# DreamScene-Project/DreamScene

Measured on AMD Instinct MI355X. Metric: fwd+bwd views/s @1024x1024, 500000 Gaussians, higher is better.
Workload: dtype f32

## Files before the change

dreamscene_amd/csrc/render.hip:

```cpp
#include "gsr_common.h"
#include <cstdlib>

namespace {

constexpr int kBatch = 256;

__device__ __forceinline__ float gsr_mul(float a, float b) {
#pragma clang fp contract(off)
  return a * b;
}
__device__ __forceinline__ float gsr_sub(float a, float b) {
#pragma clang fp contract(off)
  return a - b;
}
__device__ __forceinline__ float gsr_exp(float x) {
  const float t = gsr_mul(x, 1.44269502162933349609375f);
  const float n = __builtin_rintf(t);
  const float f = gsr_sub(t, n);
  float p = 0.001326472731307149f;
  p = __fmaf_rn(p, f, 0.009671512991189957f);
  p = __fmaf_rn(p, f, 0.05550733581185341f);
  p = __fmaf_rn(p, f, 0.24022242426872253f);
  p = __fmaf_rn(p, f, 0.6931470036506653f);
  p = __fmaf_rn(p, f, 1.0f);
  return __builtin_amdgcn_ldexpf(p, gsr_f2i_sat_fast(n));
}
__device__ __forceinline__ float gsr_power(float hA, float nB, float hC, float dx, float dy) {
  return __fmaf_rn(dx, __fmaf_rn(hA, dx, gsr_mul(nB, dy)), gsr_mul(gsr_mul(hC, dy), dy));
}

struct TilePix {
  int px, py, bx, by;
  bool inside;
};

__device__ __forceinline__ TilePix tile_pixel(int tile, int gx, int W, int H) {
  const int tid = threadIdx.x, wave = tid >> 6, lane = tid & 63;
  const int ty = tile / gx, tx = tile - ty * gx;
  TilePix p;
  p.bx = tx * GSR_TILE + (wave & 1) * 8;
  p.by = ty * GSR_TILE + (wave >> 1) * 8;
  p.px = p.bx + (lane & 7);
  p.py = p.by + (lane >> 3);
  p.inside = (p.px < W) && (p.py < H);
  return p;
}

template <int W1>
__device__ __forceinline__ bool block_reach(float A, float C, float B2, float nBiA, float nBiC, float tau, float cx,
                                            float cy, float bx, float by) {
  const float dx1 = cx - bx, dx0 = dx1 - (float)(W1 - 1), dy1 = cy - by, dy0 = dy1 - (float)(W1 - 1);
  const float ex = __builtin_amdgcn_fmed3f(dx0, 0.f, dx1), ey = __builtin_amdgcn_fmed3f(dy0, 0.f, dy1);
  const float y = __builtin_amdgcn_fmed3f(dy0, nBiC * ex, dy1);
  const float q1 = A * ex * ex + (B2 * ex + C * y) * y;
  const float x = __builtin_amdgcn_fmed3f(dx0, nBiA * ey, dx1);
  const float q2 = C * ey * ey + (B2 * ey + A * x) * x;
  return fminf(q1, q2) <= tau;
}

template <int W1>
__device__ __forceinline__ uint32_t block_mask_t(const float4 q0, const float4 q1, const float4 q2, int x0i, int y0i) {
  const float tau = q2.z;
  if (!(tau >= 0.f)) return 0u;
  const float A = q0.z, B = q0.w, C = q1.x;
  const float nBiA = -B * __builtin_amdgcn_rcpf(A), nBiC = -B * __builtin_amdgcn_rcpf(C), B2 = 2.f * B;
  const float x0 = (float)x0i, y0 = (float)y0i;
  uint32_t m = 0;
  m |= (uint32_t)block_reach<W1>(A, C, B2, nBiA, nBiC, tau, q0.x, q0.y, x0, y0);
  m |= (uint32_t)block_reach<W1>(A, C, B2, nBiA, nBiC, tau, q0.x, q0.y, x0 + (float)W1, y0) << 1;
  m |= (uint32_t)block_reach<W1>(A, C, B2, nBiA, nBiC, tau, q0.x, q0.y, x0, y0 + (float)W1) << 2;
  m |= (uint32_t)block_reach<W1>(A, C, B2, nBiA, nBiC, tau, q0.x, q0.y, x0 + (float)W1, y0 + (float)W1) << 3;
  return m;
}

template <int CTRL>
__device__ __forceinline__ int gsr_dpp_i(int v) {
  return __builtin_amdgcn_update_dpp(0, v, CTRL, 0xF, 0xF, true);
}

__device__ __forceinline__ uint32_t block_excl_scan_1024(uint32_t x, uint32_t* wave_tot, uint32_t* carry_s, bool update) {
  const int tid = threadIdx.x, lane = tid & 63, wave = tid >> 6;
  uint32_t inc = x;
#pragma unroll
  for (int o = 1; o < 64; o <<= 1) {
    const uint32_t t = (uint32_t)__shfl_up((int)inc, o, 64);
    if (lane >= o) inc += t;
  }
  if (lane == 63) wave_tot[wave] = inc;
  __syncthreads();
  uint32_t woff = 0;
  for (int w = 0; w < wave; ++w) woff += wave_tot[w];
  const uint32_t carry = *carry_s;
  const uint32_t excl = carry + woff + inc - x;
  __syncthreads();
  if (update && tid == 1023) *carry_s = carry + woff + inc;
  __syncthreads();
  return excl;
}

struct WorkFwdViews {
  const uint32_t* ranges[GSR_MAX_BATCH_VIEWS];
  uint32_t* tile_depth[GSR_MAX_BATCH_VIEWS];
  uint32_t* work[GSR_MAX_BATCH_VIEWS];
  uint32_t* stats_host[GSR_MAX_BATCH_VIEWS];
};
struct WorkBwdViews {
  const uint32_t* tile_depth[GSR_MAX_BATCH_VIEWS];
  uint32_t* items[GSR_MAX_BATCH_VIEWS];
  uint32_t items_cap[GSR_MAX_BATCH_VIEWS];
  uint32_t seg_len[GSR_MAX_BATCH_VIEWS];
};

#ifndef GSR_ORDER_FRAC_BITS
#define GSR_ORDER_FRAC_BITS 2
#endif
constexpr int kOrderFrac = GSR_ORDER_FRAC_BITS;
constexpr int kOrderClasses = 2 + (32 << kOrderFrac);
__device__ __forceinline__ uint32_t order_class(uint32_t len) {
  if (len == 0u) return 0u;
  const int msb = 31 - __clz(len);
  if constexpr (kOrderFrac == 0) return (uint32_t)msb + 1u;
  const uint32_t frac = (msb >= kOrderFrac ? (len >> (msb - kOrderFrac)) : (len << (kOrderFrac - msb))) & ((1u << kOrderFrac) - 1u);
  return 1u + ((uint32_t)msb << kOrderFrac) + frac;
}
__global__ void __launch_bounds__(1024)
k_work_order_fwd(const uint32_t n_tiles, const WorkFwdViews wv) {
  const uint32_t* __restrict__ ranges = wv.ranges[blockIdx.x];
  uint32_t* __restrict__ tile_depth = wv.tile_depth[blockIdx.x];
  uint32_t* __restrict__ work = wv.work[blockIdx.x];
  uint32_t* __restrict__ stats_host = wv.stats_host[blockIdx.x];
  __shared__ uint32_t cnt[kOrderClasses], cur[kOrderClasses];
  const int tid = threadIdx.x;
  if (tid < kOrderClasses) cnt[tid] = 0;
  __syncthreads();
  for (uint32_t t = tid; t < n_tiles; t += 1024) {
    const uint32_t len = ranges[2 * t + 1] - ranges[2 * t];
    atomicAdd(&cnt[order_class(len)], 1u);
    tile_depth[t] = 0;
  }
  __syncthreads();
  if (tid == 0) {
    uint32_t run = 0;
    for (int b = kOrderClasses - 1; b >= 0; --b) { cur[b] = run; run += cnt[b]; }
    work[n_tiles] = n_tiles - cnt[0];
    if (stats_host) *stats_host = n_tiles - cnt[0];
  }
  __syncthreads();
  for (uint32_t t = tid; t < n_tiles; t += 1024) {
    const uint32_t len = ranges[2 * t + 1] - ranges[2 * t];
    work[atomicAdd(&cur[order_class(len)], 1u)] = t;
  }
}

__global__ void __launch_bounds__(1024)
k_work_order_bwd(const uint32_t n_tiles, const WorkBwdViews wv) {
  const uint32_t* __restrict__ tile_depth = wv.tile_depth[blockIdx.x];
  uint32_t* __restrict__ items = wv.items[blockIdx.x];
  const uint32_t items_cap = wv.items_cap[blockIdx.x];
  const uint32_t kb = wv.seg_len[blockIdx.x];
  __shared__ uint32_t cnt[32], cur[32];
  const int tid = threadIdx.x;
  if (tid < 32) cnt[tid] = 0;
  __syncthreads();
  for (uint32_t t = tid; t < n_tiles; t += 1024) {
    const uint32_t d = tile_depth[t];
    if (d == 0) continue;
    const uint32_t full = d / kb, tail = d % kb;
    for (uint32_t sgi = 0; sgi < full; ++sgi) atomicAdd(&cnt[15u - min(15u, (d - kb * sgi - 1u) >> 8)], 1u);
    if (tail) atomicAdd(&cnt[16u + 15u - ((tail - 1u) * 16u) / kb], 1u);
  }
  __syncthreads();
  if (tid == 0) {
    uint32_t run = 0;
    for (int b = 0; b < 32; ++b) { cur[b] = run; run += cnt[b]; }
    items[0] = min(run, items_cap);
  }
  __syncthreads();
  for (uint32_t t = tid; t < n_tiles; t += 1024) {
    const uint32_t d = tile_depth[t];
    if (d == 0) continue;
    const uint32_t full = d / kb, tail = d % kb;
    for (uint32_t sgi = 0; sgi < full; ++sgi) {
      const uint32_t i = atomicAdd(&cur[15u - min(15u, (d - kb * sgi - 1u) >> 8)], 1u);
      if (i < items_cap) { items[2 + 2 * i] = t; items[3 + 2 * i] = sgi; }
    }
    if (tail) {
      const uint32_t i = atomicAdd(&cur[16u + 15u - ((tail - 1u) * 16u) / kb], 1u);
      if (i < items_cap) { items[2 + 2 * i] = t; items[3 + 2 * i] = full; }
    }
  }
}

template <bool SCORE, int PAD = 0>
struct Stage {
  float4 s0[2][kBatch + PAD], s1[2][kBatch + PAD], s2[2][kBatch + PAD];
  uint32_t sid[SCORE ? 2 : 1][SCORE ? kBatch : 1];
  uint32_t cnt[SCORE ? 2 : 1][SCORE ? kBatch : 1];
};
__device__ __forceinline__ uint32_t stage_mask(const float4& s2row) { return __float_as_uint(s2row.w); }

template <bool SCORE, int KB>
__device__ __forceinline__ void
render_fwd_body(const uint32_t item, const int W, const int H, const uint32_t* __restrict__ work, float* __restrict__ ckpt,
             const uint32_t* __restrict__ ranges,
             const uint32_t* __restrict__ point_list, const float4* __restrict__ splat, const float* __restrict__ bg,
             float* __restrict__ out_color, float* __restrict__ out_da, float* __restrict__ final_T,
             uint32_t* __restrict__ n_contrib, uint32_t* __restrict__ tile_depth, float* __restrict__ score,
             const int score_mode) {
  __shared__ Stage<SCORE, 1> st;
  __shared__ uint16_t cand[4][kBatch + 16];
  if (threadIdx.x < 2) {
    st.s0[threadIdx.x][kBatch] = make_float4(0.f, 0.f, 0.f, 0.f);
    st.s1[threadIdx.x][kBatch] = make_float4(0.f, 0.f, 0.f, 0.f);
    st.s2[threadIdx.x][kBatch] = make_float4(0.f, 0.f, 0.f, 0.f);
  }
  if constexpr (SCORE) { st.cnt[0][threadIdx.x] = 0u; st.cnt[1][threadIdx.x] = 0u; }
  auto flush_counts = [&](const int b) {
    if constexpr (SCORE) {
      const uint32_t c = st.cnt[b][threadIdx.x];
      if (c) {
        atomicAdd(reinterpret_cast<uint32_t*>(score) + st.sid[b][threadIdx.x], c);
        st.cnt[b][threadIdx.x] = 0u;
      }
    }
  };
  const int gx = (W + GSR_TILE - 1) / GSR_TILE;
  const int tid = threadIdx.x, wave = tid >> 6, lane = tid & 63;
  const int slot = (lane >> 2) & 3, pcol = lane & 3, prow = lane >> 4;
  const float bg0 = bg[0], bg1 = bg[1], bg2 = bg[2];
  {
    const uint32_t tile = work[item >> 2];
    const int quarter = (int)(item & 3u);
    const int ty = (int)tile / gx, tx = (int)tile - ty * gx;
    const int q_x0 = tx * GSR_TILE + (quarter & 1) * 8, q_y0 = ty * GSR_TILE + (quarter >> 1) * 8;
    const int px = q_x0 + (wave & 1) * 4 + pcol, py = q_y0 + (wave >> 1) * 4 + prow;
    const bool inside = (px < W) && (py < H);
    const float pxf = (float)px, pyf = (float)py;
    const uint32_t r0 = ranges[2 * tile], r1 = ranges[2 * tile + 1];
    if (r0 == r1) {
      if (quarter == 0) {
        const int ex = tx * GSR_TILE + (tid & 15), ey = ty * GSR_TILE + (tid >> 4);
        if (ex < W && ey < H) {
          const size_t pix = (size_t)ey * W + ex, HW = (size_t)H * W;
          final_T[pix] = 1.0f;
          n_contrib[pix] = 0u;
          out_color[pix] = bg0; out_color[HW + pix] = bg1; out_color[2 * HW + pix] = bg2;
          out_da[pix] = 0.f; out_da[HW + pix] = 0.f;
        }
      }
      return;
    }

    unsigned long long donem = __builtin_amdgcn_ballot_w64(!inside);
    float T = 1.0f, C0 = 0.f, C1 = 0.f, C2 = 0.f, Dp = 0.f, Wt = 0.f;
    uint32_t last = 0;

    uint32_t nid = 0;
    float4 n0 = make_float4(0, 0, 0, 0), n1 = n0, n2 = n0;
    if (r0 + tid < r1) {
      nid = point_list[r0 + tid];
      const float4* r = splat + 3 * (size_t)nid;
      n0 = r[0]; n1 = r[1]; n2 = r[2];
    }
    int buf = 0;
    for (uint32_t base = r0; base < r1; base += kBatch, buf ^= 1) {
      const int n = (int)min((uint32_t)kBatch, r1 - base);
      st.s0[buf][tid] = make_float4(n0.x, n0.y, -0.5f * n0.z, -n0.w);
      st.s1[buf][tid] = make_float4(-0.5f * n1.x, n1.y, n1.z, n1.w);
      st.s2[buf][tid] = make_float4(n2.x, n2.y, n2.z,
                                    __uint_as_float((tid < n) ? block_mask_t<4>(n0, n1, n2, q_x0, q_y0) : 0u));
      if constexpr (SCORE) st.sid[buf][tid] = nid;
      const int n_done = __syncthreads_count(__builtin_amdgcn_inverse_ballot_w64(donem));
      if (score_mode != 1 && base != r0) flush_counts(buf ^ 1);
      if (n_done == 256) break;
      auto checkpoint = [&](const uint32_t pos) {
        if (ckpt == nullptr) return;
        float f0 = C0, f1 = C1, f2 = C2, f3 = Dp, f4 = Wt;
        f0 += gsr_dpp<0x124>(f0); f0 += gsr_dpp<0x128>(f0);
        f1 += gsr_dpp<0x124>(f1); f1 += gsr_dpp<0x128>(f1);
        f2 += gsr_dpp<0x124>(f2); f2 += gsr_dpp<0x128>(f2);
        f3 += gsr_dpp<0x124>(f3); f3 += gsr_dpp<0x128>(f3);
        f4 += gsr_dpp<0x124>(f4); f4 += gsr_dpp<0x128>(f4);
        if (slot == 0 && inside) {
          float* ck = ckpt + (size_t)(pos / KB) * (6 * 256) + ((py - ty * GSR_TILE) * GSR_TILE + (px - tx * GSR_TILE));
          ck[0] = T; ck[256] = f0; ck[512] = f1; ck[768] = f2; ck[1024] = f3; ck[1280] = f4;
        }
      };
      if (base != r0) checkpoint(base);
      {
        const uint32_t idx = base + kBatch + tid;
        if (idx < r1) {
          nid = point_list[idx];
          const float4* r = splat + 3 * (size_t)nid;
          n0 = r[0]; n1 = r[1]; n2 = r[2];
        }
      }
      int cnt = 0;
      int cut_at[3] = {-1, -1, -1};
#pragma unroll
      for (int k = 0; k < kBatch / 64; ++k) {
        if (k * 64 >= n) break;
        const bool m = (stage_mask(st.s2[buf][k * 64 + lane]) >> wave) & 1u;
        const unsigned long long bal = __builtin_amdgcn_ballot_w64(m);
        if (m) cand[wave][cnt + (int)__builtin_amdgcn_mbcnt_hi((uint32_t)(bal >> 32), __builtin_amdgcn_mbcnt_lo((uint32_t)bal, 0u))] = (uint8_t)(k * 64 + lane);
        cnt += (int)__popcll(bal);
        if constexpr (KB < kBatch) {
          if (((k + 1) * 64) % KB == 0 && k + 1 < kBatch / 64 && (k + 1) * 64 < n) {
            const int pad = (-cnt) & 3;
            if (lane < pad) cand[wave][cnt + lane] = (uint16_t)kBatch;
            cnt += pad;
            cut_at[(k + 1) * 64 / KB - 1] = cnt;
          }
        }
      }
      if (lane < 3) cand[wave][cnt + lane] = (uint16_t)kBatch;
      __builtin_amdgcn_fence(__ATOMIC_ACQ_REL, "wavefront");
      __builtin_amdgcn_wave_barrier();
      {
        for (int i = 0;; i += 4) {
          if (donem == ~0ull) break;
          if constexpr (KB < kBatch) {
#pragma unroll
            for (int c = 0; c < kBatch / KB - 1; ++c)
              if (i == cut_at[c]) checkpoint(base + (uint32_t)((c + 1) * KB));
          }
          if (i >= cnt) break;
          const int j = (int)cand[wave][i + slot];
          const float4 a = st.s0[buf][j];
          const float4 b = st.s1[buf][j];
          const float2 c = *reinterpret_cast<const float2*>(&st.s2[buf][j]);
          const float dx = a.x - pxf, dy = a.y - pyf;
          const float power = gsr_power(a.z, a.w, b.x, dx, dy);
          const float alpha = fminf(GSR_ALPHA_MAX, gsr_mul(b.y, gsr_exp(power)));
          const unsigned long long gm = ~donem & __builtin_amdgcn_ballot_w64(power <= 0.0f) &
                                        __builtin_amdgcn_ballot_w64(alpha >= GSR_ALPHA_MIN);
          const bool g = __builtin_amdgcn_inverse_ballot_w64(gm);
          const float fgate = g ? gsr_sub(1.0f, alpha) : 1.0f;
          float test_T = gsr_mul(T, fgate);
          asm("s_nop 1\n\t"
              "v_mul_f32_dpp %0, %0, %1 row_shr:4 row_mask:0xf bank_mask:0xe\n\t"
              "s_nop 1\n\t"
              "v_mul_f32_dpp %0, %0, %1 row_shr:4 row_mask:0xf bank_mask:0xc\n\t"
              "s_nop 1\n\t"
              "v_mul_f32_dpp %0, %0, %1 row_shr:4 row_mask:0xf bank_mask:0x8"
              : "+v"(test_T) : "v"(fgate));
          float w_all = alpha * T;
          asm("s_nop 1\n\t"
              "v_mul_f32_dpp %0, %1, %2 row_shr:4 row_mask:0xf bank_mask:0xe"
              : "+v"(w_all) : "v"(test_T), "v"(alpha));
          const unsigned long long stopm = __builtin_amdgcn_ballot_w64(test_T < GSR_T_MIN);
          const bool hit = __builtin_amdgcn_inverse_ballot_w64(gm & ~stopm);
          const float w = hit ? w_all : 0.0f;
          C0 = fmaf(b.w, w, C0); C1 = fmaf(c.x, w, C1); C2 = fmaf(c.y, w, C2);
          Dp = fmaf(b.z, w, Dp);
          Wt += w;
          last = hit ? ((base - r0) + (uint32_t)j + 1u) : last;
          if constexpr (SCORE) {
            const unsigned long long hm = __ballot(hit) & (0x000F000F000F000Full << (4 * slot));
            if (score_mode != 1) {
              if (hm != 0ull && lane == 4 * slot) atomicAdd(&st.cnt[buf][j & (kBatch - 1)], (uint32_t)__popcll(hm));
            } else {
              float ws = w;
              ws += gsr_dpp<0xB1>(ws);
              ws += gsr_dpp<0x4E>(ws);
              ws += __shfl_xor(ws, 16, 64);
              ws += __shfl_xor(ws, 32, 64);
              if (hm != 0ull && lane == 4 * slot) unsafeAtomicAdd(score + st.sid[buf][j & (kBatch - 1)], ws);
            }
          }
          uint32_t tn = __float_as_uint(hit ? test_T : T);
          tn = min(tn, (uint32_t)gsr_dpp_i<0x124>((int)tn));
          tn = min(tn, (uint32_t)gsr_dpp_i<0x128>((int)tn));
          T = __uint_as_float(tn);
          unsigned long long quad_stop = (stopm >> 12) & 0x000F000F000F000Full;
          quad_stop |= quad_stop << 4;
          quad_stop |= quad_stop << 8;
          donem |= quad_stop;
        }
      }
    }
    if constexpr (SCORE) {
      __syncthreads();
      if (score_mode != 1) flush_counts(buf ^ 1);
    }
    C0 += gsr_dpp<0x124>(C0); C0 += gsr_dpp<0x128>(C0);
    C1 += gsr_dpp<0x124>(C1); C1 += gsr_dpp<0x128>(C1);
    C2 += gsr_dpp<0x124>(C2); C2 += gsr_dpp<0x128>(C2);
    Dp += gsr_dpp<0x124>(Dp); Dp += gsr_dpp<0x128>(Dp);
    Wt += gsr_dpp<0x124>(Wt); Wt += gsr_dpp<0x128>(Wt);
    {
      int l = (int)last;
      l = max(l, gsr_dpp_i<0x124>(l));
      l = max(l, gsr_dpp_i<0x128>(l));
      last = (uint32_t)l;
    }
    if (inside && slot == 0) {
      const size_t pix = (size_t)py * W + px, HW = (size_t)H * W;
      final_T[pix] = T;
      n_contrib[pix] = last;
      out_color[pix] = C0 + T * bg0;
      out_color[HW + pix] = C1 + T * bg1;
      out_color[2 * HW + pix] = C2 + T * bg2;
      out_da[pix] = Dp;
      out_da[HW + pix] = Wt;
    }
    const uint32_t wm = gsr_wave_max_u32(last);
    if (lane == 0 && wm) atomicMax(tile_depth + tile, wm);
  }
}

template <bool SCORE>
__device__ __forceinline__ void
render_fwd_tile_body(const uint32_t item, const int W, const int H, const uint32_t* __restrict__ work, float* __restrict__ ckpt,
                  const uint32_t* __restrict__ ranges, const uint32_t* __restrict__ point_list,
                  const float4* __restrict__ splat, const float* __restrict__ bg, float* __restrict__ out_color,
                  float* __restrict__ out_da, float* __restrict__ final_T, uint32_t* __restrict__ n_contrib,
                  uint32_t* __restrict__ tile_depth, float* __restrict__ score, const int score_mode) {
  __shared__ Stage<SCORE> st;
  const int gx = (W + GSR_TILE - 1) / GSR_TILE;
  const int tile = (int)work[item];
  const int tid = threadIdx.x, wave = tid >> 6, lane = tid & 63;
  const TilePix p = tile_pixel(tile, gx, W, H);
  const int tile_x0 = p.bx - (wave & 1) * 8, tile_y0 = p.by - (wave >> 1) * 8;
  const float pxf = (float)p.px, pyf = (float)p.py;
  const uint32_t r0 = ranges[2 * tile], r1 = ranges[2 * tile + 1];
  unsigned long long donem = __builtin_amdgcn_ballot_w64(!p.inside);
  float T = 1.0f, C0 = 0.f, C1 = 0.f, C2 = 0.f, Dp = 0.f, Wt = 0.f;
  uint32_t last = 0;
  uint32_t nid = 0;
  float4 n0 = make_float4(0, 0, 0, 0), n1 = n0, n2 = n0;
  if (r0 + tid < r1) {
    nid = point_list[r0 + tid];
    const float4* r = splat + 3 * (size_t)nid;
    n0 = r[0]; n1 = r[1]; n2 = r[2];
  }
  int buf = 0;
  for (uint32_t base = r0; base < r1; base += kBatch, buf ^= 1) {
    const int n = (int)min((uint32_t)kBatch, r1 - base);
    st.s0[buf][tid] = make_float4(n0.x, n0.y, -0.5f * n0.z, -n0.w);
    st.s1[buf][tid] = make_float4(-0.5f * n1.x, n1.y, n1.z, n1.w);
    st.s2[buf][tid] = make_float4(n2.x, n2.y, n2.z,
                                  __uint_as_float((tid < n) ? block_mask_t<8>(n0, n1, n2, tile_x0, tile_y0) : 0u));
    if constexpr (SCORE) st.sid[buf][tid] = nid;
    if (__syncthreads_count(__builtin_amdgcn_inverse_ballot_w64(donem)) == 256) break;
    if (base != r0 && p.inside && ckpt != nullptr) {
      float* ck = ckpt + (size_t)(base / kBatch) * (6 * 256) + ((p.py - tile_y0) * GSR_TILE + (p.px - tile_x0));
      ck[0] = T; ck[256] = C0; ck[512] = C1; ck[768] = C2; ck[1024] = Dp; ck[1280] = Wt;
    }
    {
      const uint32_t idx = base + kBatch + tid;
      if (idx < r1) {
        nid = point_list[idx];
        const float4* r = splat + 3 * (size_t)nid;
        n0 = r[0]; n1 = r[1]; n2 = r[2];
      }
    }
    for (int k = 0; k < kBatch / 64; ++k) {
      if (k * 64 >= n) break;
      unsigned long long bits = __ballot((stage_mask(st.s2[buf][k * 64 + lane]) >> wave) & 1u);
      while (bits) {
        if (donem == ~0ull) break;
        const int j = k * 64 + __builtin_ctzll(bits);
        bits &= bits - 1ull;
        const float4 a = st.s0[buf][j];
        const float4 b = st.s1[buf][j];
        const float4 c = st.s2[buf][j];
        const float dx = a.x - pxf, dy = a.y - pyf;
        const float power = gsr_power(a.z, a.w, b.x, dx, dy);
        const float alpha = fminf(GSR_ALPHA_MAX, gsr_mul(b.y, gsr_exp(power)));
        const float test_T = gsr_mul(T, gsr_sub(1.0f, alpha));
        const unsigned long long gm = ~donem & __builtin_amdgcn_ballot_w64(power <= 0.0f) &
                                      __builtin_amdgcn_ballot_w64(alpha >= GSR_ALPHA_MIN);
        const unsigned long long stopm = gm & __builtin_amdgcn_ballot_w64(test_T < GSR_T_MIN);
        donem |= stopm;
        const bool hit = __builtin_amdgcn_inverse_ballot_w64(gm & ~stopm);
        const float w = hit ? alpha * T : 0.0f;
        if constexpr (SCORE) {
          const unsigned long long hm = __ballot(hit);
          if (hm) {
            if (score_mode != 1) {
              if (lane == 0) atomicAdd(reinterpret_cast<uint32_t*>(score) + st.sid[buf][j], (uint32_t)__popcll(hm));
            } else {
              float sc = gsr_wave_sum_to_lane63(w);
              sc = __shfl(sc, 63, 64);
              if (lane == 0) unsafeAtomicAdd(score + st.sid[buf][j], sc);
            }
          }
        }
        C0 = fmaf(b.w, w, C0); C1 = fmaf(c.x, w, C1); C2 = fmaf(c.y, w, C2);
        Dp = fmaf(b.z, w, Dp);
        Wt += w;
        T = hit ? test_T : T;
        last = hit ? ((base - r0) + (uint32_t)j + 1u) : last;
      }
    }
  }
  if (p.inside) {
    const size_t pix = (size_t)p.py * W + p.px, HW = (size_t)H * W;
    final_T[pix] = T;
    n_contrib[pix] = last;
    out_color[pix] = C0 + T * bg[0];
    out_color[HW + pix] = C1 + T * bg[1];
    out_color[2 * HW + pix] = C2 + T * bg[2];
    out_da[pix] = Dp;
    out_da[HW + pix] = Wt;
  }
  const uint32_t wm = gsr_wave_max_u32(last);
  if (lane == 0 && wm) atomicMax(tile_depth + tile, wm);
}

__device__ __forceinline__ float add_swap32(float a, float b) {
  const auto r = __builtin_amdgcn_permlane32_swap(__float_as_uint(a), __float_as_uint(b), false, false);
  return __uint_as_float(r[0]) + __uint_as_float(r[1]);
}
__device__ __forceinline__ float add_swap16(float a, float b) {
  const auto r = __builtin_amdgcn_permlane16_swap(__float_as_uint(a), __float_as_uint(b), false, false);
  return __uint_as_float(r[0]) + __uint_as_float(r[1]);
}
__device__ __forceinline__ float reduce10(const float v[10], int lane) {
  float p0, p1, p2, p3, p4, q0, q1, q2;
  asm("s_nop 1\n\t"
      "v_add_f32_dpp %0, %8, %8 row_ror:8 row_mask:0xf bank_mask:0x3\n\t"
      "v_add_f32_dpp %0, %9, %9 row_ror:8 row_mask:0xf bank_mask:0xc\n\t"
      "v_add_f32_dpp %1, %10, %10 row_ror:8 row_mask:0xf bank_mask:0x3\n\t"
      "v_add_f32_dpp %1, %11, %11 row_ror:8 row_mask:0xf bank_mask:0xc\n\t"
      "v_add_f32_dpp %2, %12, %12 row_ror:8 row_mask:0xf bank_mask:0x3\n\t"
      "v_add_f32_dpp %2, %13, %13 row_ror:8 row_mask:0xf bank_mask:0xc\n\t"
      "v_add_f32_dpp %3, %14, %14 row_ror:8 row_mask:0xf bank_mask:0x3\n\t"
      "v_add_f32_dpp %3, %15, %15 row_ror:8 row_mask:0xf bank_mask:0xc\n\t"
      "v_add_f32_dpp %4, %16, %16 row_ror:8 row_mask:0xf bank_mask:0x3\n\t"
      "v_add_f32_dpp %4, %17, %17 row_ror:8 row_mask:0xf bank_mask:0xc\n\t"
      "s_nop 1\n\t"
      "v_add_f32_dpp %5, %0, %0 row_half_mirror row_mask:0xf bank_mask:0x5\n\t"
      "v_add_f32_dpp %5, %1, %1 row_half_mirror row_mask:0xf bank_mask:0xa\n\t"
      "v_add_f32_dpp %6, %2, %2 row_half_mirror row_mask:0xf bank_mask:0x5\n\t"
      "v_add_f32_dpp %6, %3, %3 row_half_mirror row_mask:0xf bank_mask:0xa\n\t"
      "v_add_f32_dpp %7, %4, %4 row_half_mirror row_mask:0xf bank_mask:0xf"
      : "=&v"(p0), "=&v"(p1), "=&v"(p2), "=&v"(p3), "=&v"(p4), "=&v"(q0), "=&v"(q1), "=&v"(q2)
      : "v"(v[0]), "v"(v[1]), "v"(v[2]), "v"(v[3]), "v"(v[4]), "v"(v[5]), "v"(v[6]), "v"(v[7]), "v"(v[8]), "v"(v[9]));
  const float r0 = add_swap32(q0, q1);
  float R = add_swap16(r0, q2);
  asm("s_nop 1\n\t"
      "v_add_f32_dpp %0, %0, %0 quad_perm:[2,3,0,1] row_mask:0xf bank_mask:0xf\n\t"
      "s_nop 1\n\t"
      "v_add_f32_dpp %0, %0, %0 quad_perm:[1,0,3,2] row_mask:0xf bank_mask:0xf"
      : "+v"(R));
  (void)lane;
  return R;
}

template <int KB>
__device__ __forceinline__ void
render_bwd_body(const uint32_t item, const int W, const int H, const uint32_t* __restrict__ items, const uint32_t* __restrict__ tile_depth,
             const float* __restrict__ ckpt,
             const uint32_t* __restrict__ ranges, const uint32_t* __restrict__ point_list,
             const float4* __restrict__ splat, const float* __restrict__ bg, const float* __restrict__ color,
             const float* __restrict__ depth_alpha, const float* __restrict__ final_T,
             const uint32_t* __restrict__ n_contrib, const float* __restrict__ dL_dcolor,
             const float* __restrict__ dL_dda, float* __restrict__ partials, unsigned long long* __restrict__ reach) {
  __shared__ float4 s0[KB], s1[KB], s2[KB];
  __shared__ uint32_t sid[KB], smask[KB];
  __shared__ unsigned long long hitw[KB / 64];
  const int gx = (W + GSR_TILE - 1) / GSR_TILE;
  const int tid = threadIdx.x, wave = tid >> 6, lane = tid & 63;
  if (item >= items[0]) return;
 {
  const int tile = (int)items[2 + 2 * item];
  const uint32_t seg = items[3 + 2 * item];
  const uint32_t depth = tile_depth[tile];
  const uint32_t lo = seg * KB, hi = min(lo + (uint32_t)KB, depth);
  const int n = (int)(hi - lo);

  const TilePix p = tile_pixel(tile, gx, W, H);
  const int tile_x0 = p.bx - (wave & 1) * 8, tile_y0 = p.by - (wave >> 1) * 8;
  const float pxf = (float)p.px, pyf = (float)p.py;
  const uint32_t r0 = ranges[2 * tile];
  const size_t pix = (size_t)p.py * W + p.px, HW = (size_t)H * W;

  const float zref = reinterpret_cast<const float*>(splat + 3 * (size_t)point_list[r0 + (hi - 1u)] + 1)[2];
  {
    float4 n0 = make_float4(0, 0, 0, 0), n1 = n0, n2 = make_float4(0, 0, -1.f, -1.f);
    uint32_t nid = 0;
    if (tid < n) {
      nid = point_list[r0 + (hi - 1u - (uint32_t)tid)];
      const float4* r = splat + 3 * (size_t)nid;
      n0 = r[0]; n1 = r[1]; n2 = r[2];
    }
    if (tid < KB) {
      s0[tid] = make_float4(n0.x, n0.y, -0.5f * n0.z, -n0.w);
      s1[tid] = make_float4(-0.5f * n1.x, n1.y, n1.z - zref, n1.w);
      s2[tid] = n2;
      sid[tid] = nid;
      smask[tid] = (tid < n) ? block_mask_t<8>(n0, n1, n2, tile_x0, tile_y0) : 0u;
    }
    if (tid < KB / 64) hitw[tid] = 0ull;
  }

  const float Tf = p.inside ? final_T[pix] : 0.f;
  const uint32_t last = p.inside ? n_contrib[pix] : 0u;
  float gC0 = 0.f, gC1 = 0.f, gC2 = 0.f, gD = 0.f, gA = 0.f;
  if (p.inside) {
    gC0 = dL_dcolor[pix]; gC1 = dL_dcolor[HW + pix]; gC2 = dL_dcolor[2 * HW + pix];
    gD = dL_dda[pix]; gA = dL_dda[HW + pix];
  }
  const float bg0 = bg[0], bg1 = bg[1], bg2 = bg[2];
  const float bg_dot = (bg0 * gC0 + bg1 * gC1) + bg2 * gC2;

  float T = Tf;
  float R = 0.f, A = 0.f;
  if (last > hi) {
    const float* ck = ckpt + (size_t)((r0 + hi) / KB) * (6 * 256) + ((p.py - tile_y0) * GSR_TILE + (p.px - tile_x0));
    const float Tc = ck[0];
    const float inv = 1.0f / Tc;
    T = Tc;
    const float rc0 = ((color[pix] - Tf * bg0) - ck[256]) * inv;
    const float rc1 = ((color[HW + pix] - Tf * bg1) - ck[512]) * inv;
    const float rc2 = ((color[2 * HW + pix] - Tf * bg2) - ck[768]) * inv;
    const float rec_z = (depth_alpha[pix] - ck[1024]) * inv;
    const float rec_a = (depth_alpha[HW + pix] - ck[1280]) * inv;
    R = rc0 * gC0 + rc1 * gC1 + rc2 * gC2 + (rec_z - zref * rec_a) * gD;
    A = rec_a;
  }
  const float cshift = zref * gD + gA;

  const int b2 = (lane >> 2) & 1, b3 = (lane >> 3) & 1, b4 = (lane >> 4) & 1, b5 = (lane >> 5) & 1;
  const int comp = b4 ? 8 + 2 * b5 + b3 : (b3 | (b2 << 1) | (b5 << 2));
  const bool commit = ((lane & 3) == 0) && !(b4 && b2);
  __syncthreads();

  for (int k = 0; k < KB / 64; ++k) {
    if (k * 64 >= n) break;
    unsigned long long bits = __ballot((smask[k * 64 + lane] >> wave) & 1u);
    unsigned long long hitk = 0ull;
    while (bits) {
      const int jb = __builtin_ctzll(bits);
      const int j = k * 64 + jb;
      bits &= bits - 1ull;
      const uint32_t pos = hi - 1u - (uint32_t)j;
      const unsigned long long livem = __builtin_amdgcn_ballot_w64(pos < last);
      if (livem == 0ull) continue;
      const float4 a = s0[j];
      const float4 b = s1[j];
      const float dx = a.x - pxf, dy = a.y - pyf;
      const float power = gsr_power(a.z, a.w, b.x, dx, dy);
      const float G = gsr_exp(power);
      const float alpha = fminf(GSR_ALPHA_MAX, gsr_mul(b.y, G));
      const unsigned long long hitm = livem & __builtin_amdgcn_ballot_w64(power <= 0.0f) &
                                      __builtin_amdgcn_ballot_w64(alpha >= GSR_ALPHA_MIN);
      if (hitm == 0ull) continue;
      hitk |= 1ull << jb;
      const bool hit = __builtin_amdgcn_inverse_ballot_w64(hitm);
      float qv = 0.f, wv = 0.f, gdl = 0.f;
      if (hit) {
        const float4 c = s2[j];
        const float inv = __builtin_amdgcn_rcpf(1.0f - alpha);
        T = T * inv;
        const float w = alpha * T;
        const float sdot = b.w * gC0 + c.x * gC1 + c.y * gC2 + b.z * gD;
        const float t1 = 1.0f - A;
        float dL_dalpha = ((sdot - R) + cshift * t1) * T;
        dL_dalpha -= (Tf * inv) * bg_dot;
        R = alpha * sdot + (1.0f - alpha) * R;
        A = __fmaf_rn(alpha, t1, A);
        qv = (b.y * dL_dalpha) * G;
        gdl = G * dL_dalpha;
        wv = w;
      }
      float v[10];
      {
        const float u = __fmaf_rn(a.z + a.z, dx, gsr_mul(a.w, dy)), w2 = __fmaf_rn(b.x + b.x, dy, gsr_mul(a.w, dx));
        const float m1 = qv * u, m2 = qv * w2;
        v[0] = m1; v[1] = m2;
        v[2] = m1 * u; v[3] = m1 * w2; v[4] = m2 * w2;
        v[5] = gdl;
        v[6] = wv * gC0; v[7] = wv * gC1; v[8] = wv * gC2;
        v[9] = wv * gD;
      }
      const float sred = reduce10(v, lane);
      if (commit) unsafeAtomicAdd(reinterpret_cast<double*>(partials) + (GSR_PARTIAL_WORDS / 2) * (size_t)sid[j] + comp, (double)sred);
    }
    if (reach && hitk && lane == 0) atomicOr(&hitw[k], hitk);
  }
  if (reach) {
    __syncthreads();
    if (tid < n && ((hitw[tid >> 6] >> (tid & 63)) & 1ull)) atomicOr(reach + (sid[tid] >> 6), 1ull << (sid[tid] & 63u));
  }
 }
}


}

static int persistent_groups(int per_cu) {
  static int cus[64] = {0};
  int dev = 0;
  if (hipGetDevice(&dev) != hipSuccess || dev < 0 || dev >= 64) dev = 0;
  if (cus[dev] == 0) {
    hipDeviceProp_t p;
    cus[dev] = (hipGetDeviceProperties(&p, dev) == hipSuccess && p.multiProcessorCount > 0) ? p.multiProcessorCount : 256;
  }
  return cus[dev] * per_cu;
}

struct FwdViews {
  const uint32_t* work[GSR_MAX_BATCH_VIEWS];
  float* ckpt[GSR_MAX_BATCH_VIEWS];
  const uint32_t* ranges[GSR_MAX_BATCH_VIEWS];
  const uint32_t* point_list[GSR_MAX_BATCH_VIEWS];
  const float4* splat[GSR_MAX_BATCH_VIEWS];
  const float* bg[GSR_MAX_BATCH_VIEWS];
  float* out_color[GSR_MAX_BATCH_VIEWS];
  float* out_da[GSR_MAX_BATCH_VIEWS];
  float* final_T[GSR_MAX_BATCH_VIEWS];
  uint32_t* n_contrib[GSR_MAX_BATCH_VIEWS];
  uint32_t* tile_depth[GSR_MAX_BATCH_VIEWS];
  float* score[GSR_MAX_BATCH_VIEWS];
};
struct BwdViews {
  const uint32_t* items[GSR_MAX_BATCH_VIEWS];
  const uint32_t* tile_depth[GSR_MAX_BATCH_VIEWS];
  const float* ckpt[GSR_MAX_BATCH_VIEWS];
  const uint32_t* ranges[GSR_MAX_BATCH_VIEWS];
  const uint32_t* point_list[GSR_MAX_BATCH_VIEWS];
  const float4* splat[GSR_MAX_BATCH_VIEWS];
  const float* bg[GSR_MAX_BATCH_VIEWS];
  const float* color[GSR_MAX_BATCH_VIEWS];
  const float* depth_alpha[GSR_MAX_BATCH_VIEWS];
  const float* final_T[GSR_MAX_BATCH_VIEWS];
  const uint32_t* n_contrib[GSR_MAX_BATCH_VIEWS];
  const float* dL_dcolor[GSR_MAX_BATCH_VIEWS];
  const float* dL_dda[GSR_MAX_BATCH_VIEWS];
  float* partials[GSR_MAX_BATCH_VIEWS];
  unsigned long long* reach[GSR_MAX_BATCH_VIEWS];
};

template <bool SCORE, int KB = kBatch>
__global__ void __launch_bounds__(256)
k_render_fwd(const int W, const int H, const FwdViews fv, const int score_mode, const uint32_t n_views,
             const uint32_t per_view) {
  const uint32_t item = per_view ? blockIdx.x % per_view : blockIdx.x / n_views;
  const int y = (int)(per_view ? blockIdx.x / per_view : blockIdx.x - item * n_views);
  render_fwd_body<SCORE, KB>(item, W, H, fv.work[y], fv.ckpt[y], fv.ranges[y], fv.point_list[y], fv.splat[y], fv.bg[y],
                         fv.out_color[y], fv.out_da[y], fv.final_T[y], fv.n_contrib[y], fv.tile_depth[y], fv.score[y],
                         score_mode);
}
template <bool SCORE>
__global__ void __launch_bounds__(256)
k_render_fwd_tile(const int W, const int H, const FwdViews fv, const int score_mode, const uint32_t n_views,
                  const uint32_t per_view) {
  const uint32_t item = per_view ? blockIdx.x % per_view : blockIdx.x / n_views;
  const int y = (int)(per_view ? blockIdx.x / per_view : blockIdx.x - item * n_views);
  render_fwd_tile_body<SCORE>(item, W, H, fv.work[y], fv.ckpt[y], fv.ranges[y], fv.point_list[y], fv.splat[y], fv.bg[y],
                              fv.out_color[y], fv.out_da[y], fv.final_T[y], fv.n_contrib[y], fv.tile_depth[y],
                              fv.score[y], score_mode);
}
template <int KB = kBatch>
__global__ void __launch_bounds__(256)
k_render_bwd(const int W, const int H, const BwdViews bv, const uint32_t n_views, const uint32_t per_view) {
  const uint32_t item = per_view ? blockIdx.x % per_view : blockIdx.x / n_views;
  const int y = (int)(per_view ? blockIdx.x / per_view : blockIdx.x - item * n_views);
  render_bwd_body<KB>(item, W, H, bv.items[y], bv.tile_depth[y], bv.ckpt[y], bv.ranges[y], bv.point_list[y], bv.splat[y], bv.bg[y],
                  bv.color[y], bv.depth_alpha[y], bv.final_T[y], bv.n_contrib[y], bv.dL_dcolor[y], bv.dL_dda[y],
                  bv.partials[y], bv.reach[y]);
}

int gsr_launch_work_order_fwd(int n, const GsrView* views, const GsrBinning* bs, const GsrImages* imgs, hipStream_t stream) {
  const uint32_t tiles = gsr_num_tiles(views[0].image_height, views[0].image_width);
  WorkFwdViews wv = WorkFwdViews{};
  for (int k = 0; k < n; ++k) {
    wv.ranges[k] = bs[k].ranges; wv.tile_depth[k] = imgs[k].tile_depth; wv.work[k] = bs[k].tile_work;
    wv.stats_host[k] = bs[k].stats_host;
  }
  hipLaunchKernelGGL(k_work_order_fwd, dim3((uint32_t)n), dim3(1024), 0, stream, tiles, wv);
  GSR_HIP(hipGetLastError());
  return GSR_OK;
}
int gsr_launch_work_order_bwd(int n, const GsrView* views, const GsrBinning* bs, const GsrImages* imgs, hipStream_t stream) {
  const uint32_t tiles = gsr_num_tiles(views[0].image_height, views[0].image_width);
  WorkBwdViews wv = WorkBwdViews{};
  for (int k = 0; k < n; ++k) {
    wv.tile_depth[k] = imgs[k].tile_depth; wv.items[k] = bs[k].tile_work + tiles; wv.items_cap[k] = bs[k].bwd_items_cap;
    wv.seg_len[k] = gsr_seg_len(bs[k]);
  }
  hipLaunchKernelGGL(k_work_order_bwd, dim3((uint32_t)n), dim3(1024), 0, stream, tiles, wv);
  GSR_HIP(hipGetLastError());
  return GSR_OK;
}

struct ScoreViews {
  float* score[GSR_MAX_BATCH_VIEWS];
  const float* splat[GSR_MAX_BATCH_VIEWS];
  const int32_t* radii[GSR_MAX_BATCH_VIEWS];
};
namespace {
__global__ void __launch_bounds__(256) k_score_finalize(const ScoreViews sv, const int32_t P) {
  const int32_t i = (int32_t)(blockIdx.x * 256u + threadIdx.x);
  if (i >= P) return;
  float* sc = sv.score[blockIdx.y];
  const uint32_t c = reinterpret_cast<const uint32_t*>(sc)[i];
  sc[i] = (c && sv.radii[blockIdx.y][i] > 0) ? sv.splat[blockIdx.y][12 * (size_t)i + 5] * (float)c : 0.0f;
}
}

int gsr_launch_render_fwd_views(int n, const GsrView* views, const GsrGeom* geoms, const GsrBinning* bs, GsrImages* imgs,
                                hipStream_t stream, GsrProfile* prof) {
  const GsrView& v = views[0];
  const uint32_t tiles = gsr_num_tiles(v.image_height, v.image_width);
  FwdViews fv = FwdViews{};
  for (int k = 0; k < n; ++k) {
    fv.work[k] = bs[k].tile_work; fv.ckpt[k] = imgs[k].ckpt; fv.ranges[k] = bs[k].ranges;
    fv.point_list[k] = bs[k].point_list; fv.splat[k] = reinterpret_cast<const float4*>(geoms[k].splat);
    fv.bg[k] = views[k].bg; fv.out_color[k] = imgs[k].color; fv.out_da[k] = imgs[k].depth_alpha;
    fv.final_T[k] = imgs[k].final_T; fv.n_contrib[k] = imgs[k].n_contrib; fv.tile_depth[k] = imgs[k].tile_depth;
    fv.score[k] = imgs[k].important_score;
  }
  const bool score = imgs[0].important_score != nullptr;
  const uint32_t ny = (uint32_t)n;
  GsrStageTimer timer(prof, stream, GSR_STAGE_RENDER_FWD);
  if (bs[0].fwd_mode == 1) {
    if (score) hipLaunchKernelGGL(k_render_fwd_tile<true>, dim3(tiles * ny), dim3(256), 0, stream, v.image_width, v.image_height, fv, v.score_mode, ny, tiles);
    else hipLaunchKernelGGL(k_render_fwd_tile<false>, dim3(tiles * ny), dim3(256), 0, stream, v.image_width, v.image_height, fv, 0, ny, tiles);
  } else {
#define GSR_LAUNCH_K6(SC, KB) hipLaunchKernelGGL((k_render_fwd<SC, KB>), dim3(tiles * 4 * ny), dim3(256), 0, stream, v.image_width, v.image_height, fv, (SC) ? v.score_mode : 0, ny, 0u)
    const uint32_t kb = gsr_seg_len(bs[0]);
    if (score) { if (kb == 64) GSR_LAUNCH_K6(true, 64); else if (kb == 128) GSR_LAUNCH_K6(true, 128); else GSR_LAUNCH_K6(true, 256); }
    else { if (kb == 64) GSR_LAUNCH_K6(false, 64); else if (kb == 128) GSR_LAUNCH_K6(false, 128); else GSR_LAUNCH_K6(false, 256); }
#undef GSR_LAUNCH_K6
  }
  GSR_HIP(hipGetLastError());
  timer.stop();
  if (score && v.score_mode == 0 && v.P > 0) {
    ScoreViews sv = ScoreViews{};
    for (int k = 0; k < n; ++k) { sv.score[k] = imgs[k].important_score; sv.splat[k] = geoms[k].splat; sv.radii[k] = geoms[k].radii; }
    hipLaunchKernelGGL(k_score_finalize, dim3(((uint32_t)v.P + 255u) / 256u, ny), dim3(256), 0, stream, sv, v.P);
    GSR_HIP(hipGetLastError());
  }
  return GSR_OK;
}
int gsr_launch_render_fwd(const GsrView& v, const GsrGeom& geom, const GsrBinning& b, GsrImages& img,
                          hipStream_t stream, GsrProfile* prof) {
  return gsr_launch_render_fwd_views(1, &v, &geom, &b, &img, stream, prof);
}

int gsr_launch_render_bwd_views(int n, const GsrView* views, const GsrGeom* geoms, const GsrBinning* bs,
                                const GsrImages* imgs, const GsrImageGrads* igs, GsrGrads* outs, hipStream_t stream,
                                GsrProfile* prof) {
  const GsrView& v = views[0];
  const uint32_t tiles = gsr_num_tiles(v.image_height, v.image_width);
  BwdViews bv = BwdViews{};
  uint32_t items_cap = 0;
  for (int k = 0; k < n; ++k) {
    bv.items[k] = bs[k].tile_work + tiles; bv.tile_depth[k] = imgs[k].tile_depth; bv.ckpt[k] = imgs[k].ckpt;
    bv.ranges[k] = bs[k].ranges; bv.point_list[k] = bs[k].point_list;
    bv.splat[k] = reinterpret_cast<const float4*>(geoms[k].splat); bv.bg[k] = views[k].bg; bv.color[k] = imgs[k].color;
    bv.depth_alpha[k] = imgs[k].depth_alpha; bv.final_T[k] = imgs[k].final_T; bv.n_contrib[k] = imgs[k].n_contrib;
    bv.dL_dcolor[k] = igs[k].dL_dcolor; bv.dL_dda[k] = igs[k].dL_ddepth_alpha; bv.partials[k] = outs[k].partials;
    bv.reach[k] = reinterpret_cast<unsigned long long*>(outs[k].reach);
    items_cap = bs[k].bwd_items_cap > items_cap ? bs[k].bwd_items_cap : items_cap;
  }
  GsrStageTimer timer(prof, stream, GSR_STAGE_RENDER_BWD);
#define GSR_LAUNCH_K7(KB) hipLaunchKernelGGL(k_render_bwd<KB>, dim3(items_cap * (uint32_t)n), dim3(256), 0, stream, v.image_width, v.image_height, bv, (uint32_t)n, bs[0].fwd_mode == 1 ? items_cap : 0u)
  const uint32_t kb = gsr_seg_len(bs[0]);
  if (kb == 64) GSR_LAUNCH_K7(64); else if (kb == 128) GSR_LAUNCH_K7(128); else GSR_LAUNCH_K7(256);
#undef GSR_LAUNCH_K7
  GSR_HIP(hipGetLastError());
  return GSR_OK;
}
int gsr_launch_render_bwd(const GsrView& v, const GsrGeom& geom, const GsrBinning& b, const GsrImages& img,
                          const GsrImageGrads& ig, GsrGrads& out, hipStream_t stream, GsrProfile* prof) {
  return gsr_launch_render_bwd_views(1, &v, &geom, &b, &img, &ig, &out, stream, prof);
}
```

Measured before the change: 5024.

## Move empty-tile background fill into work-order kernel with vectorized stores

```diff
diff --git a/dreamscene_amd/csrc/render.hip b/dreamscene_amd/csrc/render.hip
--- a/dreamscene_amd/csrc/render.hip
+++ b/dreamscene_amd/csrc/render.hip
@@ -103,6 +103,12 @@
   uint32_t* tile_depth[GSR_MAX_BATCH_VIEWS];
   uint32_t* work[GSR_MAX_BATCH_VIEWS];
   uint32_t* stats_host[GSR_MAX_BATCH_VIEWS];
+  const float* bg[GSR_MAX_BATCH_VIEWS];
+  float* out_color[GSR_MAX_BATCH_VIEWS];
+  float* out_da[GSR_MAX_BATCH_VIEWS];
+  float* final_T[GSR_MAX_BATCH_VIEWS];
+  uint32_t* n_contrib[GSR_MAX_BATCH_VIEWS];
+  uint8_t whole_tile[GSR_MAX_BATCH_VIEWS];
 };
 struct WorkBwdViews {
   const uint32_t* tile_depth[GSR_MAX_BATCH_VIEWS];
@@ -123,8 +129,55 @@
   const uint32_t frac = (msb >= kOrderFrac ? (len >> (msb - kOrderFrac)) : (len << (kOrderFrac - msb))) & ((1u << kOrderFrac) - 1u);
   return 1u + ((uint32_t)msb << kOrderFrac) + frac;
 }
+__device__ __forceinline__ void fill_empty_tiles(const uint32_t n_tiles, const uint32_t n_views, const int W, const int H,
+                                                 const bool vec, const WorkFwdViews& wv) {
+  const int gx = (W + GSR_TILE - 1) / GSR_TILE;
+  const int lane = threadIdx.x & 63;
+  const uint32_t wave = (uint32_t)__builtin_amdgcn_readfirstlane((int)(threadIdx.x >> 6));
+  const uint32_t n_waves = (gridDim.x - n_views) * 16u, total = n_tiles * n_views;
+  const size_t HW = (size_t)H * W;
+  for (uint32_t u = (blockIdx.x - n_views) * 16u + wave; u < total; u += n_waves) {
+    const uint32_t y = u / n_tiles, t = u - y * n_tiles;
+    const uint32_t* __restrict__ ranges = wv.ranges[y];
+    if (ranges[2 * t] != ranges[2 * t + 1]) continue;
+    const int ty = (int)t / gx, tx = (int)t - ty * gx;
+    const int ex = tx * GSR_TILE + (lane & 3) * 4, ey = ty * GSR_TILE + (lane >> 2);
+    const int n = min(4, W - ex);
+    if (ey >= H || n <= 0) continue;
+    const float* __restrict__ bg = wv.bg[y];
+    float c0 = bg[0], c1 = bg[1], c2 = bg[2];
+    if (wv.whole_tile[y]) { c0 = 0.f + c0; c1 = 0.f + c1; c2 = 0.f + c2; }
+    const size_t pix = (size_t)ey * W + ex;
+    float* __restrict__ col = wv.out_color[y] + pix;
+    float* __restrict__ da = wv.out_da[y] + pix;
+    float* __restrict__ fT = wv.final_T[y] + pix;
+    uint32_t* __restrict__ nc = wv.n_contrib[y] + pix;
+    if (vec) {
+      *reinterpret_cast<float4*>(fT) = make_float4(1.0f, 1.0f, 1.0f, 1.0f);
+      *reinterpret_cast<uint4*>(nc) = make_uint4(0u, 0u, 0u, 0u);
+      *reinterpret_cast<float4*>(col) = make_float4(c0, c0, c0, c0);
+      *reinterpret_cast<float4*>(col + HW) = make_float4(c1, c1, c1, c1);
+      *reinterpret_cast<float4*>(col + 2 * HW) = make_float4(c2, c2, c2, c2);
+      *reinterpret_cast<float4*>(da) = make_float4(0.f, 0.f, 0.f, 0.f);
+      *reinterpret_cast<float4*>(da + HW) = make_float4(0.f, 0.f, 0.f, 0.f);
+    } else {
+      for (int k = 0; k < n; ++k) {
+        fT[k] = 1.0f;
+        nc[k] = 0u;
+        col[k] = c0; col[HW + k] = c1; col[2 * HW + k] = c2;
+        da[k] = 0.f; da[HW + k] = 0.f;
+      }
+    }
+  }
+}
+
 __global__ void __launch_bounds__(1024)
-k_work_order_fwd(const uint32_t n_tiles, const WorkFwdViews wv) {
+k_work_order_fwd(const uint32_t n_tiles, const WorkFwdViews wv, const uint32_t n_views, const int W, const int H,
+                 const int vec) {
+  if (blockIdx.x >= n_views) {
+    fill_empty_tiles(n_tiles, n_views, W, H, vec != 0, wv);
+    return;
+  }
   const uint32_t* __restrict__ ranges = wv.ranges[blockIdx.x];
   uint32_t* __restrict__ tile_depth = wv.tile_depth[blockIdx.x];
   uint32_t* __restrict__ work = wv.work[blockIdx.x];
@@ -237,19 +290,7 @@
     const bool inside = (px < W) && (py < H);
     const float pxf = (float)px, pyf = (float)py;
     const uint32_t r0 = ranges[2 * tile], r1 = ranges[2 * tile + 1];
-    if (r0 == r1) {
-      if (quarter == 0) {
-        const int ex = tx * GSR_TILE + (tid & 15), ey = ty * GSR_TILE + (tid >> 4);
-        if (ex < W && ey < H) {
-          const size_t pix = (size_t)ey * W + ex, HW = (size_t)H * W;
-          final_T[pix] = 1.0f;
-          n_contrib[pix] = 0u;
-          out_color[pix] = bg0; out_color[HW + pix] = bg1; out_color[2 * HW + pix] = bg2;
-          out_da[pix] = 0.f; out_da[HW + pix] = 0.f;
-        }
-      }
-      return;
-    }
+    if (r0 == r1) return;
 
     unsigned long long donem = __builtin_amdgcn_ballot_w64(!inside);
     float T = 1.0f, C0 = 0.f, C1 = 0.f, C2 = 0.f, Dp = 0.f, Wt = 0.f;
@@ -424,6 +465,7 @@
   const int tile_x0 = p.bx - (wave & 1) * 8, tile_y0 = p.by - (wave >> 1) * 8;
   const float pxf = (float)p.px, pyf = (float)p.py;
   const uint32_t r0 = ranges[2 * tile], r1 = ranges[2 * tile + 1];
+  if (r0 == r1) return;
   unsigned long long donem = __builtin_amdgcn_ballot_w64(!p.inside);
   float T = 1.0f, C0 = 0.f, C1 = 0.f, C2 = 0.f, Dp = 0.f, Wt = 0.f;
   uint32_t last = 0;
@@ -764,14 +806,25 @@
                   bv.partials[y], bv.reach[y]);
 }
 
+#ifndef GSR_FILL_PER_CU
+#define GSR_FILL_PER_CU 1
+#endif
 int gsr_launch_work_order_fwd(int n, const GsrView* views, const GsrBinning* bs, const GsrImages* imgs, hipStream_t stream) {
   const uint32_t tiles = gsr_num_tiles(views[0].image_height, views[0].image_width);
   WorkFwdViews wv = WorkFwdViews{};
+  uintptr_t low = 0;
   for (int k = 0; k < n; ++k) {
     wv.ranges[k] = bs[k].ranges; wv.tile_depth[k] = imgs[k].tile_depth; wv.work[k] = bs[k].tile_work;
     wv.stats_host[k] = bs[k].stats_host;
-  }
-  hipLaunchKernelGGL(k_work_order_fwd, dim3((uint32_t)n), dim3(1024), 0, stream, tiles, wv);
+    wv.bg[k] = views[k].bg; wv.out_color[k] = imgs[k].color; wv.out_da[k] = imgs[k].depth_alpha;
+    wv.final_T[k] = imgs[k].final_T; wv.n_contrib[k] = imgs[k].n_contrib; wv.whole_tile[k] = bs[k].fwd_mode == 1;
+    low |= (uintptr_t)imgs[k].color | (uintptr_t)imgs[k].depth_alpha | (uintptr_t)imgs[k].final_T | (uintptr_t)imgs[k].n_contrib;
+  }
+  const int W = views[0].image_width, H = views[0].image_height;
+  const int vec = ((low & 15u) == 0 && W % 4 == 0) ? 1 : 0;
+  const uint32_t fill_max = (uint32_t)persistent_groups(GSR_FILL_PER_CU), fill_need = (tiles * (uint32_t)n + 15u) / 16u;
+  const uint32_t fill = fill_need < fill_max ? fill_need : fill_max;
+  hipLaunchKernelGGL(k_work_order_fwd, dim3((uint32_t)n + fill), dim3(1024), 0, stream, tiles, wv, (uint32_t)n, W, H, vec);
   GSR_HIP(hipGetLastError());
   return GSR_OK;
 }
```

New measurement: 5006. About the same (-0.4%).
